# OpenHardware-Initiative/Drone-OA-IREE-ViT-Accelerator

Hardware: AMD Instinct MI355X
Metric: frames/s on ITAViTLSTM int8, 60x90 depth input (higher is better)
Workload: dtype int8+f32; 1 GPU; ITAViTLSTM int8 end-to-end forward (BASELINE config 4): 1024 synthetic 60x90 depth frames per GPU per step, LSTM state carried, velocity all-gather; frames_per_gpu=1024, global_batch=1024, parallelism=dp1, image_dtype=u8, weights=seed-0 synthetic QAT (tests/golden), gather_every=1, gather=none (one GPU), schedule=one stream

## Files before the change

drone-oa-iree-vit-accelerator_amd/csrc/ita_f16x3_kernels.h:

```cpp
#pragma once
#include <type_traits>
#include "ita_device.h"

typedef _Float16 f16x8 __attribute__((ext_vector_type(8)));
typedef _Float16 f16x4 __attribute__((ext_vector_type(4)));
typedef float f32x16 __attribute__((ext_vector_type(16)));
typedef unsigned u32x2 __attribute__((ext_vector_type(2)));
typedef unsigned u32x4 __attribute__((ext_vector_type(4)));

__device__ __forceinline__ __amdgpu_buffer_rsrc_t ita_rsrc(const void* p) {
  return __builtin_amdgcn_make_buffer_rsrc(const_cast<void*>(p), (short)0, 0x7FFFFFFF, 0x00020000);
}
constexpr int ITA_SC1 = 16;

__device__ __forceinline__ void split_f16(float x, _Float16& hi, _Float16& lo) {
  hi = (_Float16)x;
  lo = (_Float16)(x - (float)hi);
}

struct ItaGemmSplitArgs {
  const _Float16 *a_hi, *a_lo; int lda;
  const _Float16 *w_hi, *w_lo; int ldw;
  float* out;
  int M, N, K;
  int nsplit;
  int dbg;
  const _Float16 *wf_hi, *wf_lo;
};

template <int ROWS, int NT>
__device__ __forceinline__ void stage_plane(const _Float16* __restrict__ g, int ld, int row0, int max_row, int k0,
                                            char* lds_plane, int tid) {
  static_assert(ROWS * 8 % NT == 0, "pieces must divide evenly over the workgroup");
#pragma unroll
  for (int p = 0; p < ROWS * 8 / NT; ++p) {
    const int piece = p * NT + tid;
    const int r = piece >> 3, s = piece & 7;
    const int c = s ^ ((r >> 1) & 7);
    const int gr = min(row0 + r, max_row);
    const _Float16* src = g + (size_t)gr * ld + k0 + c * 8;
    char* dst = lds_plane + (p * NT + (tid & ~63)) * 16;
    __builtin_amdgcn_global_load_lds((const __attribute__((address_space(1))) void*)src,
                                     (__attribute__((address_space(3))) void*)dst, 16, 0, 0);
  }
}

__device__ __forceinline__ f16x8 frag_f16(const char* lds_plane, int r, int chunk) {
  return *(const f16x8*)(lds_plane + r * 128 + ((chunk ^ ((r >> 1) & 7)) << 4));
}

template <int BM, int BN>
struct ItaGemmSplitLds {
  static constexpr int A_PLANE = BM * 128, W_PLANE = BN * 128;
  static constexpr int BUF = 2 * A_PLANE + 2 * W_PLANE;
  static constexpr int TOTAL = 2 * BUF;
};

template <int BM, int BN, int WM, int WN>
__global__ __launch_bounds__(64 * WM * WN) void ita_gemm_f16x3_kernel(const ItaGemmSplitArgs g) {
  using L = ItaGemmSplitLds<BM, BN>;
  constexpr int NT = 64 * WM * WN;
  constexpr int TM = BM / (32 * WM), TN = BN / (32 * WN);
  extern __shared__ __attribute__((aligned(16))) char lds[];
  const int tid = threadIdx.x, lane = tid & 63, wave = tid >> 6;
  const int wm = wave / WN, wn = wave % WN;
  const int bid = blockIdx.x;
  const int zsplit = bid % g.nsplit, tile = bid / g.nsplit;
  const int ntn = g.N / BN;
  const int m0 = (tile / ntn) * BM, n0 = (tile % ntn) * BN;
  const int kslice = g.K / g.nsplit, kbeg = zsplit * kslice;
  const int nt = kslice / 64;
  const int r = lane & 31, h = lane >> 5;

  f32x16 acc[TM][TN];
#pragma unroll
  for (int i = 0; i < TM; ++i)
#pragma unroll
    for (int j = 0; j < TN; ++j)
#pragma unroll
      for (int e = 0; e < 16; ++e) acc[i][j][e] = 0.0f;

  auto stage = [&](int buf, int t) {
    char* b = lds + buf * L::BUF;
    const int k0 = kbeg + t * 64;
    const int m0s = (g.dbg & 16) ? 0 : m0, n0s = (g.dbg & 32) ? 0 : n0, k0s = (g.dbg & 64) ? t * 64 : k0;
    stage_plane<BM, NT>(g.a_hi, g.lda, m0s, g.M - 1, k0s, b, tid);
    stage_plane<BM, NT>(g.a_lo, g.lda, m0s, g.M - 1, k0s, b + L::A_PLANE, tid);
    stage_plane<BN, NT>(g.w_hi, g.ldw, n0s, g.N - 1, k0s, b + 2 * L::A_PLANE, tid);
    stage_plane<BN, NT>(g.w_lo, g.ldw, n0s, g.N - 1, k0s, b + 2 * L::A_PLANE + L::W_PLANE, tid);
  };

  auto compute = [&](int buf) {
    const char* b = lds + buf * L::BUF;
    const char *ah = b, *al = b + L::A_PLANE, *wh = b + 2 * L::A_PLANE, *wl = wh + L::W_PLANE;
#pragma unroll
    for (int ks = 0; ks < 4; ++ks) {
      f16x8 fah[TM], fal[TM], fwh[TN], fwl[TN];
#pragma unroll
      for (int i = 0; i < TM; ++i) {
        const int row = wm * (BM / WM) + i * 32 + r;
        fah[i] = frag_f16(ah, row, 2 * ks + h);
        fal[i] = frag_f16(al, row, 2 * ks + h);
      }
#pragma unroll
      for (int j = 0; j < TN; ++j) {
        const int row = wn * (BN / WN) + j * 32 + r;
        fwh[j] = frag_f16(wh, row, 2 * ks + h);
        fwl[j] = frag_f16(wl, row, 2 * ks + h);
      }
#pragma unroll
      for (int i = 0; i < TM; ++i)
#pragma unroll
        for (int j = 0; j < TN; ++j) {
          acc[i][j] = __builtin_amdgcn_mfma_f32_32x32x16_f16(fal[i], fwh[j], acc[i][j], 0, 0, 0);
          acc[i][j] = __builtin_amdgcn_mfma_f32_32x32x16_f16(fah[i], fwl[j], acc[i][j], 0, 0, 0);
          acc[i][j] = __builtin_amdgcn_mfma_f32_32x32x16_f16(fah[i], fwh[j], acc[i][j], 0, 0, 0);
        }
    }
  };
  int cur = 0;
  stage(0, 0);
  __syncthreads();
  for (int t = 0; t < nt; ++t) {
    if (t + 1 < nt && !(g.dbg & 2)) stage(cur ^ 1, t + 1);
    if (!(g.dbg & 1)) compute(g.dbg & 8 ? 0 : cur);
    if (!(g.dbg & 4)) __syncthreads();
    cur ^= 1;
  }
  float* out = g.out + (size_t)zsplit * g.M * g.N;
#pragma unroll
  for (int i = 0; i < TM; ++i)
#pragma unroll
    for (int j = 0; j < TN; ++j) {
      const int n = n0 + wn * (BN / WN) + j * 32 + r;
#pragma unroll
      for (int e = 0; e < 16; ++e) {
        const int m = m0 + wm * (BM / WM) + i * 32 + (e & 3) + 8 * (e >> 2) + 4 * h;
        if (m < g.M) __hip_atomic_store(out + (size_t)m * g.N + n, acc[i][j][e], __ATOMIC_RELAXED, __HIP_MEMORY_SCOPE_AGENT);
      }
    }
}

constexpr int ITA_GEMM_SMALL_NSTG = 3;
constexpr int ita_gemm_small_lds(int mt) { return ITA_GEMM_SMALL_NSTG * (2 * mt + 2) * 32 * 128; }
constexpr int ita_waitcnt_vm(int n) { return (n & 15) | ((n >> 4) << 14) | 0x0F70; }
template <int MT>
__global__ __launch_bounds__(256) void ita_gemm_f16x3_small_kernel(const ItaGemmSplitArgs g) {
  constexpr int NSTG = ITA_GEMM_SMALL_NSTG, PLANE = 32 * 128, APL = MT * PLANE, STG = 2 * APL + 2 * PLANE;
  constexpr int DMA = 2 * MT + 2;
  static_assert(NSTG == 3 && DMA < 64, "one younger k-tile in flight at the wait; vmcnt range");
  extern __shared__ __attribute__((aligned(16))) char lds[];
  const int tid = threadIdx.x, lane = tid & 63, wave = __builtin_amdgcn_readfirstlane(tid >> 6), r = lane & 31, h = lane >> 5;
  const int z = blockIdx.x % g.nsplit, n0 = (blockIdx.x / g.nsplit) * 32, m0 = blockIdx.y * 32 * MT;
  const int kslice = g.K / g.nsplit, kbeg = z * kslice, nt = kslice / 64;
  auto stage = [&](int kt, int slot) {
    char* b = lds + slot * STG;
    const int k0 = kbeg + kt * 64;
    stage_plane<32 * MT, 256>(g.a_hi, g.lda, m0, g.M - 1, k0, b, tid);
    stage_plane<32 * MT, 256>(g.a_lo, g.lda, m0, g.M - 1, k0, b + APL, tid);
    stage_plane<32, 256>(g.w_hi, g.ldw, n0, g.N - 1, k0, b + 2 * APL, tid);
    stage_plane<32, 256>(g.w_lo, g.ldw, n0, g.N - 1, k0, b + 2 * APL + PLANE, tid);
  };
#pragma unroll
  for (int s = 0; s < NSTG - 1; ++s)
    if (s < nt) stage(s, s);
  f32x16 acc;
#pragma unroll
  for (int e = 0; e < 16; ++e) acc[e] = 0.0f;
  const bool compute = wave < MT && m0 + 32 * wave < g.M;
  for (int kt = 0; kt < nt; ++kt) {
    if (kt + 1 < nt) __builtin_amdgcn_s_waitcnt(ita_waitcnt_vm(DMA)); else __builtin_amdgcn_s_waitcnt(ita_waitcnt_vm(0));
    __builtin_amdgcn_s_waitcnt(0xC07F);
    __builtin_amdgcn_s_barrier();
    asm volatile("" ::: "memory");
    __builtin_amdgcn_sched_barrier(0);
    if (kt + NSTG - 1 < nt) stage(kt + NSTG - 1, (kt + NSTG - 1) % NSTG);
    if (compute) {
      const char* b = lds + (kt % NSTG) * STG;
      const char *pah = b + wave * PLANE, *pal = b + APL + wave * PLANE, *pwh = b + 2 * APL, *pwl = pwh + PLANE;
#pragma unroll
      for (int ks = 0; ks < 4; ++ks) {
        const f16x8 ah = frag_f16(pah, r, 2 * ks + h), al = frag_f16(pal, r, 2 * ks + h);
        const f16x8 wh = frag_f16(pwh, r, 2 * ks + h), wl = frag_f16(pwl, r, 2 * ks + h);
        acc = __builtin_amdgcn_mfma_f32_32x32x16_f16(al, wh, acc, 0, 0, 0);
        acc = __builtin_amdgcn_mfma_f32_32x32x16_f16(ah, wl, acc, 0, 0, 0);
        acc = __builtin_amdgcn_mfma_f32_32x32x16_f16(ah, wh, acc, 0, 0, 0);
      }
    }
  }
  if (!compute) return;
  float* out = g.out + (size_t)z * g.M * g.N;
#pragma unroll
  for (int e = 0; e < 16; ++e) {
    const int m = m0 + 32 * wave + (e & 3) + 8 * (e >> 2) + 4 * h;
    if (m < g.M) out[(size_t)m * g.N + n0 + r] = acc[e];
  }
}

__global__ __launch_bounds__(64) void ita_gemm_f16x3_tiny_kernel(const ItaGemmSplitArgs g) {
  const int lane = threadIdx.x, r = lane & 31, h = lane >> 5;
  const int n0 = blockIdx.x * 32, m0 = blockIdx.y * 32, z = blockIdx.z;
  const int kslice = g.K / g.nsplit, kbeg = z * kslice, nstep = kslice / 16;
  const size_t ao = (size_t)min(m0 + r, g.M - 1) * g.lda + kbeg + 8 * h;
  const size_t wo = (((size_t)blockIdx.x * (g.K / 16) + kbeg / 16) * 64 + lane) * 8;
  constexpr int R = 8;
  f16x8 ah[R], al[R], wh[R], wl[R];
  auto fetch = [&](int s, int slot) {
    ah[slot] = *(const f16x8*)(g.a_hi + ao + 16 * s);
    al[slot] = *(const f16x8*)(g.a_lo + ao + 16 * s);
    wh[slot] = *(const f16x8*)(g.wf_hi + wo + (size_t)s * 512);
    wl[slot] = *(const f16x8*)(g.wf_lo + wo + (size_t)s * 512);
  };
#pragma unroll
  for (int s = 0; s < R; ++s) fetch(s, s);
  f32x16 acc;
#pragma unroll
  for (int e = 0; e < 16; ++e) acc[e] = 0.0f;
  for (int s0 = 0; s0 < nstep; s0 += R) {
#pragma unroll
    for (int j = 0; j < R; ++j) {
      acc = __builtin_amdgcn_mfma_f32_32x32x16_f16(al[j], wh[j], acc, 0, 0, 0);
      acc = __builtin_amdgcn_mfma_f32_32x32x16_f16(ah[j], wl[j], acc, 0, 0, 0);
      acc = __builtin_amdgcn_mfma_f32_32x32x16_f16(ah[j], wh[j], acc, 0, 0, 0);
      if (s0 + R + j < nstep) fetch(s0 + R + j, j);
    }
  }
  float* out = g.out + (size_t)z * g.M * g.N;
#pragma unroll
  for (int e = 0; e < 16; ++e) {
    const int m = m0 + (e & 3) + 8 * (e >> 2) + 4 * h;
    if (m < g.M) out[(size_t)m * g.N + n0 + r] = acc[e];
  }
}

__device__ __forceinline__ size_t ita_lstm_plane_index(int b, int k) {
  return ((size_t)(((b >> 5) * 4 + (k >> 6)) * 4 + ((k >> 4) & 3)) * 64 + ((k >> 3) & 1) * 32 + (b & 31)) * 8 + (k & 7);
}
__device__ __forceinline__ float lstm_sigmoid_fast(float x) {
  return __builtin_amdgcn_rcpf(1.0f + __builtin_amdgcn_exp2f(x * -1.44269504088896341f));
}
__device__ __forceinline__ float lstm_tanh_fast(float x) {
  return 1.0f - 2.0f * __builtin_amdgcn_rcpf(__builtin_amdgcn_exp2f(x * 2.88539008177792681f) + 1.0f);
}
struct ItaLstmHeadArgs {
  const float* part; float inv_fold_scale;
  const _Float16 *w0_hi, *w0_lo; float inv_wscale0;
  const float* bias0;
  const _Float16 *w1_hi, *w1_lo, *w2_hi, *w2_lo;
  float inv_wscale1, inv_wscale2;
  const float *bsum1, *bsum2;
  const float *desvel, *quat;
  const float *h_in, *c_in;
  float *h_out, *c_out;
  size_t lstride;
  _Float16 *p1_hi, *p1_lo, *p2_hi, *p2_lo;
  const float *fc_w, *fc_b; float* vel;
  unsigned *cnt, *err;
  int B;
  const int* slots;
};
constexpr int ITA_HEAD_CNT_STRIDE = 64;
constexpr unsigned ITA_HEAD_ERR_TIMEOUT = 1;
constexpr unsigned long long ITA_HEAD_SPIN_TICKS = 200000000ull;
__device__ __forceinline__ f16x8 ita_load_sc1_f16x8(const _Float16* base, int byte_off) {
  return __builtin_bit_cast(f16x8, __builtin_amdgcn_raw_buffer_load_b128(ita_rsrc(base), byte_off, 0, ITA_SC1));
}
__device__ __forceinline__ bool ita_head_poll(unsigned* cnt, unsigned target, unsigned* err) {
  const unsigned long long t0 = wall_clock64();
  while (__hip_atomic_load(cnt, __ATOMIC_RELAXED, __HIP_MEMORY_SCOPE_AGENT) < target) {
    if (wall_clock64() - t0 > ITA_HEAD_SPIN_TICKS) {
      __hip_atomic_fetch_or(err, ITA_HEAD_ERR_TIMEOUT, __ATOMIC_RELAXED, __HIP_MEMORY_SCOPE_AGENT);
      return false;
    }
    __builtin_amdgcn_s_sleep(2);
  }
  return true;
}
template <int NS>
__global__ __launch_bounds__(256, 2) void ita_lstm_head_kernel(const ItaLstmHeadArgs a) {
  __shared__ __attribute__((aligned(16))) float big[32 * 132 + 32 * 36];
  __shared__ __attribute__((aligned(16))) f16x8 hin[2][2][4][2][64];
  __shared__ __attribute__((aligned(16))) _Float16 pub[2][32][8];
  __shared__ unsigned flag;
  float (*hs)[132] = (float (*)[132])big;
  float (*pt)[36] = (float (*)[36])(big + 32 * 132);
  float (*part)[16][64] = (float (*)[16][64])big;
  const int tid = threadIdx.x, lane = tid & 63, wave = __builtin_amdgcn_readfirstlane(tid >> 6);
  const int ft = blockIdx.x >> 4, ut = blockIdx.x & 15, f0 = ft * 32;
  const int r = lane & 31, h = lane >> 5;
  const int B = a.B;
  const int ef = tid >> 3, eu = tid & 7;
  int rh[4], rb0 = min(f0 + r, B - 1), reb = min(f0 + ef, B - 1);
#pragma unroll
  for (int i = 0; i < 4; ++i) rh[i] = min(f0 + 2 * (4 * wave + i) + h, B - 1);
  if (a.slots) {
#pragma unroll
    for (int i = 0; i < 4; ++i) rh[i] = a.slots[rh[i]];
    rb0 = a.slots[rb0];
    reb = a.slots[reb];
  }

  f32x4 pz[NS];
#pragma unroll
  for (int z = 0; z < NS; ++z)
    pz[z] = *(const f32x4*)(a.part + ((size_t)z * B + min(f0 + 8 * wave + (lane >> 3), B - 1)) * 512 + ut * 32 + 4 * (lane & 7));
  f32x4 hv[4];
#pragma unroll
  for (int i = 0; i < 4; ++i) hv[i] = *(const f32x4*)(a.h_in + (size_t)rh[i] * 128 + 4 * r);
  const int b0 = f0 + r, u0 = ut * 8 + 4 * h;
  const size_t sb0 = (size_t)rb0;
  if (wave >= 2) {
    f32x4 hx[2][4][2];
#pragma unroll
    for (int l = 0; l < 2; ++l)
#pragma unroll
      for (int s = 0; s < 4; ++s) {
        const float* src = a.h_in + (l + 1) * a.lstride + sb0 * 128 + 64 * (wave - 2) + 16 * s + 8 * h;
        hx[l][s][0] = *(const f32x4*)src;
        hx[l][s][1] = *(const f32x4*)(src + 4);
      }
    __builtin_amdgcn_sched_barrier(0);
#pragma unroll
    for (int l = 0; l < 2; ++l)
#pragma unroll
      for (int s = 0; s < 4; ++s) {
        f16x8 xh, xl;
#pragma unroll
        for (int j = 0; j < 8; ++j) {
          _Float16 hi, lo;
          split_f16(hx[l][s][j >> 2][j & 3], hi, lo);
          xh[j] = hi;
          xl[j] = lo;
        }
        hin[l][wave - 2][s][0][lane] = xh;
        hin[l][wave - 2][s][1][lane] = xl;
      }
  }
  f16x8 wh[9], wl[9];
  f32x4 q = {0.0f, 0.0f, 0.0f, 0.0f}, ci0 = {0.0f, 0.0f, 0.0f, 0.0f}, bz[4];
  float dv = 0.0f;
  if (wave == 0) {
    const _Float16* wfr_hi = a.w0_hi + ((size_t)ut * 9 * 64 + lane) * 8;
    const _Float16* wfr_lo = a.w0_lo + ((size_t)ut * 9 * 64 + lane) * 8;
#pragma unroll
    for (int s = 0; s < 9; ++s) {
      wh[s] = *(const f16x8*)(wfr_hi + s * 512);
      wl[s] = *(const f16x8*)(wfr_lo + s * 512);
    }
    const int bc = min(b0, B - 1);
    q = *(const f32x4*)(a.quat + (size_t)bc * 4);
    dv = a.desvel[bc];
    ci0 = *(const f32x4*)(a.c_in + sb0 * 128 + u0);
#pragma unroll
    for (int gt = 0; gt < 4; ++gt) bz[gt] = *(const f32x4*)(a.bias0 + gt * 128 + u0);
  }
  const size_t wo = ((size_t)((ut * 4 + wave) * 4) * 64 + lane) * 8;
  f16x8 w1h[4], w1l[4];
#pragma unroll
  for (int s = 0; s < 4; ++s) {
    w1h[s] = *(const f16x8*)(a.w1_hi + wo + 512 * s);
    w1l[s] = *(const f16x8*)(a.w1_lo + wo + 512 * s);
  }
  const int eb = f0 + ef, un = ut * 8 + eu;
  const size_t esb = (size_t)reb;
  const float c1_prev = a.c_in[a.lstride + esb * 128 + un], c2_prev = a.c_in[2 * a.lstride + esb * 128 + un];
  float bs1[4], bs2[4];
#pragma unroll
  for (int gt = 0; gt < 4; ++gt) {
    bs1[gt] = a.bsum1[gt * 128 + un];
    bs2[gt] = a.bsum2[gt * 128 + un];
  }
  __builtin_amdgcn_sched_barrier(0);
  {
    f32x4 ps = pz[0];
#pragma unroll
    for (int z = 1; z < NS; ++z) ps += pz[z];
    *(f32x4*)&pt[8 * wave + (lane >> 3)][4 * (lane & 7)] = ps;
  }
#pragma unroll
  for (int i = 0; i < 4; ++i) *(f32x4*)&hs[2 * (4 * wave + i) + h][4 * r] = hv[i];
  __syncthreads();

  f32x4 hn0 = {0.0f, 0.0f, 0.0f, 0.0f};
  if (wave == 0) {
    f32x16 acc;
#pragma unroll
    for (int e = 0; e < 16; ++e) acc[e] = 0.0f;
    f32x4 xlast0 = {0.0f, 0.0f, 0.0f, 0.0f};
    float xlast1 = 0.0f;
    if (h == 0) {
      xlast0 = (f32x4){dv / 10.0f, q.x, q.y, q.z};
      xlast1 = q.w;
    }
#pragma unroll
    for (int s = 0; s < 9; ++s) {
      f32x4 x0 = xlast0, x1 = {xlast1, 0.0f, 0.0f, 0.0f};
      if (s < 8) {
        x0 = *(const f32x4*)&hs[r][16 * s + 8 * h];
        x1 = *(const f32x4*)&hs[r][16 * s + 8 * h + 4];
      }
      f16x8 xh, xl;
#pragma unroll
      for (int j = 0; j < 8; ++j) {
        const float x = j < 4 ? x0[j & 3] : x1[j & 3];
        const _Float16 hi = (_Float16)x;
        xh[j] = hi;
        xl[j] = (_Float16)(x - (float)hi);
      }
      acc = __builtin_amdgcn_mfma_f32_32x32x16_f16(wl[s], xh, acc, 0, 0, 0);
      acc = __builtin_amdgcn_mfma_f32_32x32x16_f16(wh[s], xl, acc, 0, 0, 0);
      acc = __builtin_amdgcn_mfma_f32_32x32x16_f16(wh[s], xh, acc, 0, 0, 0);
    }
    f32x4 cn;
#pragma unroll
    for (int q = 0; q < 4; ++q) {
      float g[4];
#pragma unroll
      for (int gt = 0; gt < 4; ++gt)
        g[gt] = (pt[r][gt * 8 + 4 * h + q] * a.inv_fold_scale + acc[4 * gt + q] * a.inv_wscale0) + bz[gt][q];
      const float ig = lstm_sigmoid_fast(g[0]), fg = lstm_sigmoid_fast(g[1]), cg = lstm_tanh_fast(g[2]), og = lstm_sigmoid_fast(g[3]);
      const float c = fmaf(fg, ci0[q], ig * cg);
      cn[q] = c;
      hn0[q] = og * lstm_tanh_fast(c);
    }
    if (b0 < B) *(f32x4*)(a.c_out + sb0 * 128 + u0) = cn;
    f16x4 x_hi, x_lo;
#pragma unroll
    for (int q = 0; q < 4; ++q) {
      _Float16 x, y;
      split_f16(hn0[q], x, y); x_hi[q] = x; x_lo[q] = y;
    }
    const int o0 = (int)ita_lstm_plane_index(b0, u0) * 2;
    __builtin_amdgcn_raw_buffer_store_b64(__builtin_bit_cast(u32x2, x_hi), ita_rsrc(a.p1_hi), o0, 0, ITA_SC1);
    __builtin_amdgcn_raw_buffer_store_b64(__builtin_bit_cast(u32x2, x_lo), ita_rsrc(a.p1_lo), o0, 0, ITA_SC1);
  }
  asm volatile("s_waitcnt vmcnt(0)" ::: "memory");
  __syncthreads();
  if (tid == 0) __hip_atomic_fetch_add(a.cnt + ft * ITA_HEAD_CNT_STRIDE, 1u, __ATOMIC_RELAXED, __HIP_MEMORY_SCOPE_AGENT);
  f16x8 w2h[4], w2l[4];
#pragma unroll
  for (int s = 0; s < 4; ++s) {
    w2h[s] = *(const f16x8*)(a.w2_hi + wo + 512 * s);
    w2l[s] = *(const f16x8*)(a.w2_lo + wo + 512 * s);
  }

#pragma unroll
  for (int l = 1; l <= 2; ++l) {
    if (tid == 0) flag = ita_head_poll(a.cnt + ft * ITA_HEAD_CNT_STRIDE, 16u * l, a.err) ? 1u : 0u;
    __syncthreads();
    if (!flag) return;
    if (l == 1 && wave == 0 && b0 < B) *(f32x4*)(a.h_out + sb0 * 128 + u0) = hn0;
    f16x8 fah[4], fal[4];
    if (wave < 2) {
      const int ao = (((ft * 4 + wave) * 4) * 64 + lane) * 16;
      const _Float16* ph = l == 1 ? a.p1_hi : a.p2_hi;
      const _Float16* pl = l == 1 ? a.p1_lo : a.p2_lo;
#pragma unroll
      for (int s = 0; s < 4; ++s) {
        fah[s] = ita_load_sc1_f16x8(ph, ao + 1024 * s);
        fal[s] = ita_load_sc1_f16x8(pl, ao + 1024 * s);
      }
    } else {
#pragma unroll
      for (int s = 0; s < 4; ++s) {
        fah[s] = hin[l - 1][wave - 2][s][0][lane];
        fal[s] = hin[l - 1][wave - 2][s][1][lane];
      }
    }
    f32x16 acc;
#pragma unroll
    for (int e = 0; e < 16; ++e) acc[e] = 0.0f;
#pragma unroll
    for (int s = 0; s < 4; ++s) {
      const f16x8 fwh = l == 1 ? w1h[s] : w2h[s], fwl = l == 1 ? w1l[s] : w2l[s];
      acc = __builtin_amdgcn_mfma_f32_32x32x16_f16(fwl, fah[s], acc, 0, 0, 0);
      acc = __builtin_amdgcn_mfma_f32_32x32x16_f16(fwh, fal[s], acc, 0, 0, 0);
      acc = __builtin_amdgcn_mfma_f32_32x32x16_f16(fwh, fah[s], acc, 0, 0, 0);
    }
#pragma unroll
    for (int e = 0; e < 16; ++e) part[wave][e][lane] = acc[e];
    __syncthreads();
    float gsum[4];
    const int pl = ef + 32 * (eu >> 2);
#pragma unroll
    for (int gte = 0; gte < 4; ++gte) {
      const int e = 4 * gte + (eu & 3);
      gsum[gte] = ((part[0][e][pl] + part[1][e][pl]) + part[2][e][pl]) + part[3][e][pl];
    }
    const float iws = l == 1 ? a.inv_wscale1 : a.inv_wscale2;
    const float* bs = l == 1 ? bs1 : bs2;
    const float gi = gsum[0] * iws + bs[0], gf = gsum[1] * iws + bs[1], gg = gsum[2] * iws + bs[2], go = gsum[3] * iws + bs[3];
    const float ig = lstm_sigmoid_fast(gi), fg = lstm_sigmoid_fast(gf), cg = lstm_tanh_fast(gg), og = lstm_sigmoid_fast(go);
    const float c = fmaf(fg, l == 1 ? c1_prev : c2_prev, ig * cg);
    const float hn = og * lstm_tanh_fast(c);
    const size_t so = l * a.lstride + esb * 128 + un;
    if (eb < B) {
      a.c_out[so] = c;
      if (l == 1) a.h_out[so] = hn;
      else
        __builtin_amdgcn_raw_buffer_store_b32(__builtin_bit_cast(unsigned, hn), ita_rsrc(a.h_out), (int)(so * 4), 0, ITA_SC1);
    }
    if (l == 1) {
      _Float16 x, y;
      split_f16(hn, x, y);
      pub[0][ef][eu] = x;
      pub[1][ef][eu] = y;
      __syncthreads();
      if (wave == 0 && h == 0) {
        const int o = (int)ita_lstm_plane_index(f0 + r, ut * 8) * 2;
        const f16x8 vh = *(const f16x8*)&pub[0][r][0], vl = *(const f16x8*)&pub[1][r][0];
        __builtin_amdgcn_raw_buffer_store_b128(__builtin_bit_cast(u32x4, vh), ita_rsrc(a.p2_hi), o, 0, ITA_SC1);
        __builtin_amdgcn_raw_buffer_store_b128(__builtin_bit_cast(u32x4, vl), ita_rsrc(a.p2_lo), o, 0, ITA_SC1);
      }
    }
    asm volatile("s_waitcnt vmcnt(0)" ::: "memory");
    __syncthreads();
    if (tid == 0) {
      const unsigned prev = __hip_atomic_fetch_add(a.cnt + ft * ITA_HEAD_CNT_STRIDE, 1u, __ATOMIC_RELAXED, __HIP_MEMORY_SCOPE_AGENT);
      if (l == 2) flag = prev == 47u ? 1u : 0u;
    }
  }

  __syncthreads();
  if (!flag) return;
  if (tid == 0) __hip_atomic_store(a.cnt + ft * ITA_HEAD_CNT_STRIDE, 0u, __ATOMIC_RELAXED, __HIP_MEMORY_SCOPE_AGENT);
  float (*fw)[128] = (float (*)[128])(big + 32 * 132);
  int fro[4];
#pragma unroll
  for (int i = 0; i < 4; ++i) fro[i] = min(f0 + ((i * 256 + tid) >> 5), B - 1);
  if (a.slots) {
#pragma unroll
    for (int i = 0; i < 4; ++i) fro[i] = a.slots[fro[i]];
  }
  f32x4 hr[4];
#pragma unroll
  for (int i = 0; i < 4; ++i) {
    const int off = (int)((2 * a.lstride + (size_t)fro[i] * 128 + 4 * (tid & 31)) * 4);
    hr[i] = __builtin_bit_cast(f32x4, __builtin_amdgcn_raw_buffer_load_b128(ita_rsrc(a.h_out), off, 0, ITA_SC1));
  }
  const f32x4 wv = *(const f32x4*)(a.fc_w + 4 * min(tid, 95));
#pragma unroll
  for (int i = 0; i < 4; ++i) *(f32x4*)&hs[(i * 256 + tid) >> 5][4 * (tid & 31)] = hr[i];
  if (tid < 96) *(f32x4*)&fw[tid >> 5][4 * (tid & 31)] = wv;
  __syncthreads();
  if (tid < 96) {
    const int fr = tid / 3, o = tid - 3 * fr, b = f0 + fr;
    if (b < B) {
      float acc = a.fc_b[o];
      for (int k = 0; k < 128; ++k) acc = fmaf(hs[fr][k], fw[o][k], acc);
      a.vel[(size_t)b * 3 + o] = acc;
    }
  }
}

__global__ void ita_split_planes_kernel(const float* __restrict__ x, _Float16* __restrict__ hi, _Float16* __restrict__ lo,
                                        int width, int ld, int rows) {
  const size_t i8 = ((size_t)blockIdx.x * blockDim.x + threadIdx.x) * 8;
  if (i8 >= (size_t)rows * width) return;
  const size_t r = i8 / width, c = i8 - r * width;
  f16x8 vh, vl;
#pragma unroll
  for (int j = 0; j < 8; ++j) {
    _Float16 a, b;
    split_f16(x[i8 + j], a, b);
    vh[j] = a; vl[j] = b;
  }
  *(f16x8*)(hi + r * ld + c) = vh;
  *(f16x8*)(lo + r * ld + c) = vl;
}

__global__ void ita_impulse_kernel(float* x, int rows, int width, int col0) {
  const size_t idx = (size_t)blockIdx.x * blockDim.x + threadIdx.x;
  if (idx >= (size_t)rows * width) return;
  const int i = (int)(idx / width), c = (int)(idx % width);
  x[idx] = (c == col0 + i) ? 1.0f : 0.0f;
}

struct ItaTailBigArgs {
  const float* x;
  const _Float16 *w_hi, *w_lo;
  const float* bias;
  float inv_wscale;
  float* out;
  int B, E, TH, TW, CO, nchunk;
  int accumulate;
};
template <int NT, int WAVES, int TPS>
struct ItaTailBigLds {
  static constexpr int HP = (2 * WAVES + 2) * 34;
  static constexpr int A_PLANE = HP * 64;
  static constexpr int W_PLANE = TPS * NT * 16 * 64;
  static constexpr int AH = 0, AL = A_PLANE, WH = 2 * A_PLANE, WL = WH + W_PLANE;
  static constexpr int GEO_I = WL + W_PLANE;
  static constexpr int GEO_F = GEO_I + HP * 16;
  static constexpr int TOTAL = GEO_F + HP * 8;
};

template <int NT, int WAVES, int TPS>
__global__ __launch_bounds__(64 * WAVES) void ita_tail_big_kernel(const ItaTailBigArgs a) {
  using L = ItaTailBigLds<NT, WAVES, TPS>;
  static_assert(9 % TPS == 0, "taps per weight stage must divide 9");
  constexpr int W_CHUNK_HALVES = 9 * NT * 16 * 32;
  constexpr int NTHR = 64 * WAVES;
  extern __shared__ __attribute__((aligned(16))) char lds[];
  const int tid = threadIdx.x, lane = tid & 63, wave = tid >> 6;
  const int OH = 2 * a.TH, OW = 2 * a.TW, C4 = a.E / 4, CIN = C4 + a.E;
  const int tx0 = blockIdx.x * 32, ty0 = blockIdx.y * 2 * WAVES, b = blockIdx.z;
  const float* xt = a.x + (size_t)b * a.TH * a.TW * a.E;
  const float sy = (float)(a.TH - 1) / (float)(OH - 1), sx = (float)(a.TW - 1) / (float)(OW - 1);

  f32x4 acc[4][NT];
#pragma unroll
  for (int mt = 0; mt < 4; ++mt)
#pragma unroll
    for (int nt = 0; nt < NT; ++nt) acc[mt][nt] = (f32x4){0.0f, 0.0f, 0.0f, 0.0f};

  for (int p = tid; p < L::HP; p += NTHR) {
    const int hy = p / 34, hx = p - 34 * hy;
    const int y = ty0 + hy - 1, x = tx0 + hx - 1;
    const int ok = (y >= 0 && y < OH && x >= 0 && x < OW) ? 4 : 0;
    const int yc = min(max(y, 0), OH - 1), xc = min(max(x, 0), OW - 1);
    const float fy = sy * (float)yc, fx = sx * (float)xc;
    int y0 = (int)fy, x0 = (int)fx;
    if (y0 > a.TH - 1) y0 = a.TH - 1;
    if (x0 > a.TW - 1) x0 = a.TW - 1;
    const int yp = y0 < a.TH - 1 ? 2 : 0, xp = x0 < a.TW - 1 ? 1 : 0;
    *(i32x4*)(lds + L::GEO_I + p * 16) = (i32x4){(y0 * a.TW + x0) * a.E,
                                                   ((yc >> 1) * a.TW + (xc >> 1)) * a.E + 2 * (yc & 1) + (xc & 1), ok | yp | xp, 0};
    *(f32x2*)(lds + L::GEO_F + p * 8) = (f32x2){fy - (float)y0, fx - (float)x0};
  }

  for (int ch = 0; ch < a.nchunk; ++ch) {
    __syncthreads();
    auto stage_w = [&](int tap0) {
      const _Float16* gh = a.w_hi + (size_t)ch * W_CHUNK_HALVES + (size_t)tap0 * NT * 16 * 32;
      const _Float16* gl = a.w_lo + (size_t)ch * W_CHUNK_HALVES + (size_t)tap0 * NT * 16 * 32;
      for (int wc = wave; wc < L::W_PLANE / 1024; wc += WAVES) {
        const int piece = wc * 64 + lane;
        __builtin_amdgcn_global_load_lds((const __attribute__((address_space(1))) void*)(gh + piece * 8),
                                         (__attribute__((address_space(3))) void*)(lds + L::WH + wc * 1024), 16, 0, 0);
        __builtin_amdgcn_global_load_lds((const __attribute__((address_space(1))) void*)(gl + piece * 8),
                                         (__attribute__((address_space(3))) void*)(lds + L::WL + wc * 1024), 16, 0, 0);
      }
    };
    stage_w(0);
    {
      constexpr int G = 5, NITEM = L::HP * 8;
      const bool all_shuffle = ch * 32 + 31 < C4, all_up = ch * 32 >= C4;
      for (int i0 = tid; i0 < NITEM; i0 += NTHR * G) {
        f32x4 q00[G], q01[G], q10[G], q11[G];
        f32x2 hw[G];
        int item[G];
        bool ok[G];
#pragma unroll
        for (int g = 0; g < G; ++g) {
          const int i = min(i0 + NTHR * g, NITEM - 1);
          const int p = i >> 3, cq = i & 7;
          const int c0 = ch * 32 + 4 * cq;
          const i32x4 gi = *(const i32x4*)(lds + L::GEO_I + p * 16);
          hw[g] = *(const f32x2*)(lds + L::GEO_F + p * 8);
          item[g] = i;
          ok[g] = i0 + NTHR * g < NITEM && (gi.z & 4) && c0 < CIN;
          if (all_shuffle || (!all_up && c0 < C4)) {
            const float* t = xt + gi.y + 4 * min(c0, C4 - 4);
            q00[g] = (f32x4){t[0], t[4], t[8], t[12]};
            q01[g] = q10[g] = q11[g] = (f32x4){0.0f, 0.0f, 0.0f, 0.0f};
          } else {
            const float* t00 = xt + gi.x + min(max(c0 - C4, 0), a.E - 4);
            const int dx = (gi.z & 1) ? a.E : 0, dy = (gi.z & 2) ? a.TW * a.E : 0;
            q00[g] = *(const f32x4*)t00;
            q01[g] = *(const f32x4*)(t00 + dx);
            q10[g] = *(const f32x4*)(t00 + dy);
            q11[g] = *(const f32x4*)(t00 + dy + dx);
          }
        }
#pragma unroll
        for (int g = 0; g < G; ++g) {
          if (i0 + NTHR * g < NITEM) {
            const int p = item[g] >> 3, cq = item[g] & 7;
            const bool shuf = all_shuffle || (!all_up && ch * 32 + 4 * cq < C4);
            const float h1 = hw[g].x, h0 = 1.0f - h1, w1 = hw[g].y, w0 = 1.0f - w1;
            f16x4 vh, vl;
#pragma unroll
            for (int j = 0; j < 4; ++j) {
              float v = shuf ? q00[g][j] : h0 * (w0 * q00[g][j] + w1 * q01[g][j]) + h1 * (w0 * q10[g][j] + w1 * q11[g][j]);
              if (!ok[g]) v = 0.0f;
              _Float16 hq, lq;
              split_f16(v, hq, lq);
              vh[j] = hq; vl[j] = lq;
            }
            *(f16x4*)(lds + L::AH + p * 64 + cq * 8) = vh;
            *(f16x4*)(lds + L::AL + p * 64 + cq * 8) = vl;
          }
        }
      }
    }
    __syncthreads();
    const int px = lane & 15, kg = lane >> 4;
#pragma unroll 1
    for (int tap = 0; tap < 9; ++tap) {
      if (TPS < 9 && tap > 0 && tap % TPS == 0) {
        __syncthreads();
        stage_w(tap);
        __syncthreads();
      }
      const int ky = tap / 3, kx = tap - 3 * ky, tl = tap % TPS;
      f16x8 bh[NT], bl[NT];
#pragma unroll
      for (int nt = 0; nt < NT; ++nt) {
        const int off = ((tl * NT * 16 + nt * 16 + px) * 64) + kg * 16;
        bh[nt] = *(const f16x8*)(lds + L::WH + off);
        bl[nt] = *(const f16x8*)(lds + L::WL + off);
      }
#pragma unroll
      for (int mt = 0; mt < 4; ++mt) {
        const int hp = (2 * wave + (mt >> 1) + ky) * 34 + (mt & 1) * 16 + px + kx;
        const f16x8 ah = *(const f16x8*)(lds + L::AH + hp * 64 + kg * 16);
        const f16x8 al = *(const f16x8*)(lds + L::AL + hp * 64 + kg * 16);
#pragma unroll
        for (int nt = 0; nt < NT; ++nt) {
          acc[mt][nt] = __builtin_amdgcn_mfma_f32_16x16x32_f16(al, bh[nt], acc[mt][nt], 0, 0, 0);
          acc[mt][nt] = __builtin_amdgcn_mfma_f32_16x16x32_f16(ah, bl[nt], acc[mt][nt], 0, 0, 0);
          acc[mt][nt] = __builtin_amdgcn_mfma_f32_16x16x32_f16(ah, bh[nt], acc[mt][nt], 0, 0, 0);
        }
      }
    }
  }
  const int co_l = lane & 15, m0 = 4 * (lane >> 4);
#pragma unroll
  for (int mt = 0; mt < 4; ++mt) {
    const int y = ty0 + 2 * wave + (mt >> 1), x = tx0 + (mt & 1) * 16 + m0;
#pragma unroll
    for (int nt = 0; nt < NT; ++nt) {
      const int co = nt * 16 + co_l;
      if (co < a.CO) {
        const float bv = a.accumulate ? 0.0f : a.bias[co];
        float* op = a.out + (((size_t)b * a.CO + co) * OH + y) * OW + x;
        f32x4 o = a.accumulate ? *(const f32x4*)op : (f32x4){0.0f, 0.0f, 0.0f, 0.0f};
#pragma unroll
        for (int i = 0; i < 4; ++i) o[i] = o[i] + (acc[mt][nt][i] * a.inv_wscale + bv);
        *(f32x4*)op = o;
      }
    }
  }
}

struct ItaTailUpArgs {
  const float* x;
  const _Float16 *w_hi, *w_lo;
  const _Float16 *s_hi, *s_lo;
  const float* bias;
  float inv_wscale;
  float* out;
  int B, TH, TW, CO;
};
struct ItaTailUpLds {
  static constexpr int RH = 10, RW = 18, NTOK = 192;
  static constexpr int YLD = 52;
  static constexpr int YB = NTOK * YLD * 4;
  static constexpr int Y = 0;
  static constexpr int WPL = 4 * 3 * 1024;
  static constexpr int W = 2 * YB;
  static constexpr int TOTAL1 = W + 2 * 2 * WPL;
  static constexpr int HP = 18 * 34, A_PLANE = HP * 64, W2_PLANE = 9 * 48 * 64;
  static constexpr int TOTAL = 160 * 1024;
  static constexpr int WL2 = TOTAL - W2_PLANE, WH2 = WL2 - W2_PLANE;
  static_assert(WL2 >= TOTAL1 && WH2 >= W + 2 * WPL && 2 * A_PLANE <= WH2 && 48 * 516 * 4 <= WH2, "phase-2 LDS");
};

#ifdef ITA_UP_STAMP
__device__ unsigned long long ita_up_stamp_buf[2048 * 8 * 12];
#define ITA_UP_ST(i) do { if (lane == 0 && tile < 2048) ita_up_stamp_buf[((size_t)tile * 8 + wave) * 12 + (i)] = __builtin_amdgcn_s_memrealtime(); } while (0)
#else
#define ITA_UP_ST(i) do { } while (0)
#endif
__global__ __launch_bounds__(512) __attribute__((amdgpu_waves_per_eu(2, 2))) void ita_tail_up_kernel(const ItaTailUpArgs a) {
  using L = ItaTailUpLds;
  constexpr int E = 128;
  extern __shared__ __attribute__((aligned(16))) char lds[];
  int tid = threadIdx.x, lane = tid & 63;
  const int wave = __builtin_amdgcn_readfirstlane(tid >> 6);
  const int OH = 2 * a.TH, OW = 2 * a.TW;
  const float sy = (float)(a.TH - 1) / (float)(OH - 1), sx = (float)(a.TW - 1) / (float)(OW - 1);
  const int tiles_x = OW / 32, tiles_y = OH / 16, ntiles = tiles_x * tiles_y * a.B;
  int tx0, ty0, b, ry0, rx0;
  const float* xt;
  auto src = [](int q, float s, int n, int& i0, int& ip, float& l1) {
    const float f = s * (float)q;
    int i = (int)f;
    if (i > n - 1) i = n - 1;
// ... 299 lines not shown
```

Before: 11.29 million frames/s.

## Precompute recurrent-state MFMA partials before the inter-block poll in LSTM head

Waves 2-3 now run the h_in-dependent MFMA partial products for LSTM layers 1 and 2 before the cross-block spin-wait, storing f32 accumulators in a new shared 'early' buffer. After the wait only waves 0-1 do MFMA work. The register array sv is shared between wave 0's w0 weights and waves 2-3's inputs and w2 weights, and the partial-sum loads are issued later. This takes MFMA work off the serialized post-barrier critical path, at the cost of more register pressure and a larger shared-memory footprint.

Measured after the change: 11.32 million frames/s, median of 6. Within noise of the previous version (+0.3%).

```diff
diff --git a/drone-oa-iree-vit-accelerator_amd/csrc/ita_f16x3_kernels.h b/drone-oa-iree-vit-accelerator_amd/csrc/ita_f16x3_kernels.h
--- a/drone-oa-iree-vit-accelerator_amd/csrc/ita_f16x3_kernels.h
+++ b/drone-oa-iree-vit-accelerator_amd/csrc/ita_f16x3_kernels.h
@@ -279,7 +279,7 @@
 template <int NS>
 __global__ __launch_bounds__(256, 2) void ita_lstm_head_kernel(const ItaLstmHeadArgs a) {
   __shared__ __attribute__((aligned(16))) float big[32 * 132 + 32 * 36];
-  __shared__ __attribute__((aligned(16))) f16x8 hin[2][2][4][2][64];
+  __shared__ __attribute__((aligned(16))) float early[2][2][16][64];
   __shared__ __attribute__((aligned(16))) _Float16 pub[2][32][8];
   __shared__ unsigned flag;
   float (*hs)[132] = (float (*)[132])big;
@@ -298,45 +298,15 @@
     for (int i = 0; i < 4; ++i) rh[i] = a.slots[rh[i]];
     rb0 = a.slots[rb0];
     reb = a.slots[reb];
-  }
-
-  f32x4 pz[NS];
-#pragma unroll
-  for (int z = 0; z < NS; ++z)
-    pz[z] = *(const f32x4*)(a.part + ((size_t)z * B + min(f0 + 8 * wave + (lane >> 3), B - 1)) * 512 + ut * 32 + 4 * (lane & 7));
+    __builtin_amdgcn_s_waitcnt(ita_waitcnt_vm(0));
+  }
+
   f32x4 hv[4];
 #pragma unroll
   for (int i = 0; i < 4; ++i) hv[i] = *(const f32x4*)(a.h_in + (size_t)rh[i] * 128 + 4 * r);
   const int b0 = f0 + r, u0 = ut * 8 + 4 * h;
   const size_t sb0 = (size_t)rb0;
-  if (wave >= 2) {
-    f32x4 hx[2][4][2];
-#pragma unroll
-    for (int l = 0; l < 2; ++l)
-#pragma unroll
-      for (int s = 0; s < 4; ++s) {
-        const float* src = a.h_in + (l + 1) * a.lstride + sb0 * 128 + 64 * (wave - 2) + 16 * s + 8 * h;
-        hx[l][s][0] = *(const f32x4*)src;
-        hx[l][s][1] = *(const f32x4*)(src + 4);
-      }
-    __builtin_amdgcn_sched_barrier(0);
-#pragma unroll
-    for (int l = 0; l < 2; ++l)
-#pragma unroll
-      for (int s = 0; s < 4; ++s) {
-        f16x8 xh, xl;
-#pragma unroll
-        for (int j = 0; j < 8; ++j) {
-          _Float16 hi, lo;
-          split_f16(hx[l][s][j >> 2][j & 3], hi, lo);
-          xh[j] = hi;
-          xl[j] = lo;
-        }
-        hin[l][wave - 2][s][0][lane] = xh;
-        hin[l][wave - 2][s][1][lane] = xl;
-      }
-  }
-  f16x8 wh[9], wl[9];
+  f32x4 sv[24];
   f32x4 q = {0.0f, 0.0f, 0.0f, 0.0f}, ci0 = {0.0f, 0.0f, 0.0f, 0.0f}, bz[4];
   float dv = 0.0f;
   if (wave == 0) {
@@ -344,8 +314,8 @@
     const _Float16* wfr_lo = a.w0_lo + ((size_t)ut * 9 * 64 + lane) * 8;
 #pragma unroll
     for (int s = 0; s < 9; ++s) {
-      wh[s] = *(const f16x8*)(wfr_hi + s * 512);
-      wl[s] = *(const f16x8*)(wfr_lo + s * 512);
+      sv[2 * s] = *(const f32x4*)(wfr_hi + s * 512);
+      sv[2 * s + 1] = *(const f32x4*)(wfr_lo + s * 512);
     }
     const int bc = min(b0, B - 1);
     q = *(const f32x4*)(a.quat + (size_t)bc * 4);
@@ -354,12 +324,29 @@
 #pragma unroll
     for (int gt = 0; gt < 4; ++gt) bz[gt] = *(const f32x4*)(a.bias0 + gt * 128 + u0);
   }
+  if (wave >= 2) {
+#pragma unroll
+    for (int l = 0; l < 2; ++l)
+#pragma unroll
+      for (int s = 0; s < 4; ++s) {
+        const float* src = a.h_in + (l + 1) * a.lstride + sb0 * 128 + 64 * (wave - 2) + 16 * s + 8 * h;
+        sv[8 * l + 2 * s] = *(const f32x4*)src;
+        sv[8 * l + 2 * s + 1] = *(const f32x4*)(src + 4);
+      }
+  }
   const size_t wo = ((size_t)((ut * 4 + wave) * 4) * 64 + lane) * 8;
   f16x8 w1h[4], w1l[4];
 #pragma unroll
   for (int s = 0; s < 4; ++s) {
     w1h[s] = *(const f16x8*)(a.w1_hi + wo + 512 * s);
     w1l[s] = *(const f16x8*)(a.w1_lo + wo + 512 * s);
+  }
+  if (wave >= 2) {
+#pragma unroll
+    for (int s = 0; s < 4; ++s) {
+      sv[16 + 2 * s] = *(const f32x4*)(a.w2_hi + wo + 512 * s);
+      sv[16 + 2 * s + 1] = *(const f32x4*)(a.w2_lo + wo + 512 * s);
+    }
   }
   const int eb = f0 + ef, un = ut * 8 + eu;
   const size_t esb = (size_t)reb;
@@ -370,22 +357,19 @@
     bs1[gt] = a.bsum1[gt * 128 + un];
     bs2[gt] = a.bsum2[gt * 128 + un];
   }
+  f32x4 pz[NS];
+#pragma unroll
+  for (int z = 0; z < NS; ++z)
+    pz[z] = *(const f32x4*)(a.part + ((size_t)z * B + min(f0 + 8 * wave + (lane >> 3), B - 1)) * 512 + ut * 32 + 4 * (lane & 7));
   __builtin_amdgcn_sched_barrier(0);
-  {
-    f32x4 ps = pz[0];
-#pragma unroll
-    for (int z = 1; z < NS; ++z) ps += pz[z];
-    *(f32x4*)&pt[8 * wave + (lane >> 3)][4 * (lane & 7)] = ps;
-  }
+
 #pragma unroll
   for (int i = 0; i < 4; ++i) *(f32x4*)&hs[2 * (4 * wave + i) + h][4 * r] = hv[i];
   __syncthreads();
-
-  f32x4 hn0 = {0.0f, 0.0f, 0.0f, 0.0f};
+  f32x16 acc0;
   if (wave == 0) {
-    f32x16 acc;
-#pragma unroll
-    for (int e = 0; e < 16; ++e) acc[e] = 0.0f;
+#pragma unroll
+    for (int e = 0; e < 16; ++e) acc0[e] = 0.0f;
     f32x4 xlast0 = {0.0f, 0.0f, 0.0f, 0.0f};
     float xlast1 = 0.0f;
     if (h == 0) {
@@ -407,17 +391,55 @@
         xh[j] = hi;
         xl[j] = (_Float16)(x - (float)hi);
       }
-      acc = __builtin_amdgcn_mfma_f32_32x32x16_f16(wl[s], xh, acc, 0, 0, 0);
-      acc = __builtin_amdgcn_mfma_f32_32x32x16_f16(wh[s], xl, acc, 0, 0, 0);
-      acc = __builtin_amdgcn_mfma_f32_32x32x16_f16(wh[s], xh, acc, 0, 0, 0);
-    }
+      const f16x8 wh = __builtin_bit_cast(f16x8, sv[2 * s]), wl = __builtin_bit_cast(f16x8, sv[2 * s + 1]);
+      acc0 = __builtin_amdgcn_mfma_f32_32x32x16_f16(wl, xh, acc0, 0, 0, 0);
+      acc0 = __builtin_amdgcn_mfma_f32_32x32x16_f16(wh, xl, acc0, 0, 0, 0);
+      acc0 = __builtin_amdgcn_mfma_f32_32x32x16_f16(wh, xh, acc0, 0, 0, 0);
+    }
+  }
+  if (wave >= 2) {
+#pragma unroll
+    for (int l = 0; l < 2; ++l) {
+      f32x16 acc;
+#pragma unroll
+      for (int e = 0; e < 16; ++e) acc[e] = 0.0f;
+#pragma unroll
+      for (int s = 0; s < 4; ++s) {
+        f16x8 xh, xl;
+#pragma unroll
+        for (int j = 0; j < 8; ++j) {
+          _Float16 hi, lo;
+          split_f16(sv[8 * l + 2 * s + (j >> 2)][j & 3], hi, lo);
+          xh[j] = hi;
+          xl[j] = lo;
+        }
+        const f16x8 fwh = l == 0 ? w1h[s] : __builtin_bit_cast(f16x8, sv[16 + 2 * s]);
+        const f16x8 fwl = l == 0 ? w1l[s] : __builtin_bit_cast(f16x8, sv[16 + 2 * s + 1]);
+        acc = __builtin_amdgcn_mfma_f32_32x32x16_f16(fwl, xh, acc, 0, 0, 0);
+        acc = __builtin_amdgcn_mfma_f32_32x32x16_f16(fwh, xl, acc, 0, 0, 0);
+        acc = __builtin_amdgcn_mfma_f32_32x32x16_f16(fwh, xh, acc, 0, 0, 0);
+      }
+#pragma unroll
+      for (int e = 0; e < 16; ++e) early[l][wave - 2][e][lane] = acc[e];
+    }
+  }
+  {
+    f32x4 ps = pz[0];
+#pragma unroll
+    for (int z = 1; z < NS; ++z) ps += pz[z];
+    *(f32x4*)&pt[8 * wave + (lane >> 3)][4 * (lane & 7)] = ps;
+  }
+  __syncthreads();
+
+  f32x4 hn0 = {0.0f, 0.0f, 0.0f, 0.0f};
+  if (wave == 0) {
     f32x4 cn;
 #pragma unroll
     for (int q = 0; q < 4; ++q) {
       float g[4];
 #pragma unroll
       for (int gt = 0; gt < 4; ++gt)
-        g[gt] = (pt[r][gt * 8 + 4 * h + q] * a.inv_fold_scale + acc[4 * gt + q] * a.inv_wscale0) + bz[gt][q];
+        g[gt] = (pt[r][gt * 8 + 4 * h + q] * a.inv_fold_scale + acc0[4 * gt + q] * a.inv_wscale0) + bz[gt][q];
       const float ig = lstm_sigmoid_fast(g[0]), fg = lstm_sigmoid_fast(g[1]), cg = lstm_tanh_fast(g[2]), og = lstm_sigmoid_fast(g[3]);
       const float c = fmaf(fg, ci0[q], ig * cg);
       cn[q] = c;
@@ -438,10 +460,12 @@
   __syncthreads();
   if (tid == 0) __hip_atomic_fetch_add(a.cnt + ft * ITA_HEAD_CNT_STRIDE, 1u, __ATOMIC_RELAXED, __HIP_MEMORY_SCOPE_AGENT);
   f16x8 w2h[4], w2l[4];
-#pragma unroll
-  for (int s = 0; s < 4; ++s) {
-    w2h[s] = *(const f16x8*)(a.w2_hi + wo + 512 * s);
-    w2l[s] = *(const f16x8*)(a.w2_lo + wo + 512 * s);
+  if (wave < 2) {
+#pragma unroll
+    for (int s = 0; s < 4; ++s) {
+      w2h[s] = *(const f16x8*)(a.w2_hi + wo + 512 * s);
+      w2l[s] = *(const f16x8*)(a.w2_lo + wo + 512 * s);
+    }
   }
 
 #pragma unroll
@@ -450,8 +474,8 @@
     __syncthreads();
     if (!flag) return;
     if (l == 1 && wave == 0 && b0 < B) *(f32x4*)(a.h_out + sb0 * 128 + u0) = hn0;
-    f16x8 fah[4], fal[4];
     if (wave < 2) {
+      f16x8 fah[4], fal[4];
       const int ao = (((ft * 4 + wave) * 4) * 64 + lane) * 16;
       const _Float16* ph = l == 1 ? a.p1_hi : a.p2_hi;
       const _Float16* pl = l == 1 ? a.p1_lo : a.p2_lo;
@@ -460,32 +484,26 @@
         fah[s] = ita_load_sc1_f16x8(ph, ao + 1024 * s);
         fal[s] = ita_load_sc1_f16x8(pl, ao + 1024 * s);
       }
-    } else {
+      f32x16 acc;
+#pragma unroll
+      for (int e = 0; e < 16; ++e) acc[e] = 0.0f;
 #pragma unroll
       for (int s = 0; s < 4; ++s) {
-        fah[s] = hin[l - 1][wave - 2][s][0][lane];
-        fal[s] = hin[l - 1][wave - 2][s][1][lane];
-      }
-    }
-    f32x16 acc;
-#pragma unroll
-    for (int e = 0; e < 16; ++e) acc[e] = 0.0f;
-#pragma unroll
-    for (int s = 0; s < 4; ++s) {
-      const f16x8 fwh = l == 1 ? w1h[s] : w2h[s], fwl = l == 1 ? w1l[s] : w2l[s];
-      acc = __builtin_amdgcn_mfma_f32_32x32x16_f16(fwl, fah[s], acc, 0, 0, 0);
-      acc = __builtin_amdgcn_mfma_f32_32x32x16_f16(fwh, fal[s], acc, 0, 0, 0);
-      acc = __builtin_amdgcn_mfma_f32_32x32x16_f16(fwh, fah[s], acc, 0, 0, 0);
-    }
-#pragma unroll
-    for (int e = 0; e < 16; ++e) part[wave][e][lane] = acc[e];
+        const f16x8 fwh = l == 1 ? w1h[s] : w2h[s], fwl = l == 1 ? w1l[s] : w2l[s];
+        acc = __builtin_amdgcn_mfma_f32_32x32x16_f16(fwl, fah[s], acc, 0, 0, 0);
+        acc = __builtin_amdgcn_mfma_f32_32x32x16_f16(fwh, fal[s], acc, 0, 0, 0);
+        acc = __builtin_amdgcn_mfma_f32_32x32x16_f16(fwh, fah[s], acc, 0, 0, 0);
+      }
+#pragma unroll
+      for (int e = 0; e < 16; ++e) part[wave][e][lane] = acc[e];
+    }
     __syncthreads();
     float gsum[4];
     const int pl = ef + 32 * (eu >> 2);
 #pragma unroll
     for (int gte = 0; gte < 4; ++gte) {
       const int e = 4 * gte + (eu & 3);
-      gsum[gte] = ((part[0][e][pl] + part[1][e][pl]) + part[2][e][pl]) + part[3][e][pl];
+      gsum[gte] = ((part[0][e][pl] + part[1][e][pl]) + early[l - 1][0][e][pl]) + early[l - 1][1][e][pl];
     }
     const float iws = l == 1 ? a.inv_wscale1 : a.inv_wscale2;
     const float* bs = l == 1 ? bs1 : bs2;
```
